# vb000/LookOnceToHear

Measured on AMD Instinct MI355X. Metric: frames_per_sec (5 s 16 kHz binaural clips, 625 STFT frames each, offline forward), higher is better.
Workload: dtype f32 via f16x3 split (3x fp16 MFMA per product, fp32 accumulate; ~22-bit operands, un-normalised rows scaled by a power of two before the split: any finite fp32 range); 1 GPU; BASELINE configs[2]: 32 x 5 s 16 kHz binaural clips per GPU, offline forward (configs/tsh.json separator, random-init weights); batch_per_gpu=32, global_batch=32, parallelism=utterance-dp1, gemm_mode=f16x3, tune=, batches_in_flight=1

## Files before the change

### include/lookonce_hip.h

```cpp
#ifndef LOOKONCE_HIP_H
#define LOOKONCE_HIP_H

#ifdef __cplusplus
extern "C" {
#endif

typedef void* lh_stream_t;

enum {
    LH_OK = 0,
    LH_ERR_ARG = 1,
    LH_ERR_UNSUPPORTED = 2,
    LH_ERR_LAUNCH = 3,
    LH_ERR_RANGE = 4
};

int lh_range_status(unsigned* range_flag, lh_stream_t stream);
int lh_range_flag_copy(unsigned* range_flag, void* host_pinned, lh_stream_t stream);
int lh_range_flag_clear(unsigned* range_flag, lh_stream_t stream);
int lh_selftest_fp16_subnormal(lh_stream_t stream);

enum { LH_GEMM_F32 = 0, LH_GEMM_F16X3 = 1 };

int lh_abi_version(void);

int lh_set_tuning(int key, int value);

int lh_check_config(int nfft, int hop, int n_mics, int emb_dim, int n_blocks_unused, int lstm_hidden,
                    int n_heads, int attn_window, int n_srcs, int spk_emb_dim);

int lh_stft_conv_in(const float* x, const float* conv_buf_in, float* conv_buf_out, const void* wfb_pk,
                    const void* wconv_pk, const float* bconv, float* z, int B, int T, int n_samples,
                    lh_stream_t stream);

int lh_embed_proj_ln(const float* emb, const float* w, const float* bias, const float* ln_w, const float* ln_b,
                     float* scratch, float* gain, int B, lh_stream_t stream);

int lh_ln_lstm_intra(const float* x, const float* ln_w, const float* ln_b, const void* w_pk, const float* b_sum,
                     float* h_out, int n_frames , int mode, lh_stream_t stream);

int lh_ln_lstm_inter(const float* x, const float* ln_w, const float* ln_b, const void* w_pk, const float* b_sum,
                     const float* h0, const float* c0, float* hN, float* cN, float* h_out, int B, int T, int mode,
                     lh_stream_t stream);

int lh_intra_stream(const float* x, const void* wih_pk, const float* b_sum, const float* whh, float* h_out,
                    int n_frames, lh_stream_t stream);

int lh_inter_matvec(const float* x, const void* wih_pk, const float* b_sum, const float* whh, const void* wlin_pk,
                    const float* blin, const float* h0, const float* c0, float* hN, float* cN, float* out, int B, int T,
                    lh_stream_t stream);

int lh_intra_block(const float* x, const void* w_pk, const float* b_sum, const void* wlin_pk, const float* blin,
                   float* out, int n_frames, lh_stream_t stream);

int lh_inter_block(const float* x, const void* w_pk, const float* b_sum, const void* wlin_pk, const float* blin,
                   const float* h0, const float* c0, float* hN, float* cN, float* out, int B, int T,
                   lh_stream_t stream);

int lh_linear_res(const float* h, const void* w_pk, const float* bias, const float* res, float* out, int rows,
                  int K, lh_stream_t stream);

#define LH_KV_PAD_ROWS 48

int lh_qkv_proj_ln(const float* y, const void* w_pk, const float* bias, const float* slopes, const float* lnq_w,
                   const float* lnq_b, const float* lnk_w, const float* lnk_b, const float* lnv_w,
                   const float* lnv_b, void* q, void* kx, void* vx, const int* ring_pos, int B, int T,
                   lh_stream_t stream);

int lh_qkv_proj_ln_rows(const float* y, const void* w_pk, const float* bias, const float* slopes, const float* lnq_w,
                        const float* lnq_b, const float* lnk_w, const float* lnk_b, const float* lnv_w,
                        const float* lnv_b, void* q, void* kx, void* vx, const int* write_pos, int B,
                        lh_stream_t stream);

int lh_local_attn(const void* q, const void* kx, const void* vx, float* merged, int B, int T, lh_stream_t stream);

int lh_ring_pack(const float* k_buf, const float* v_buf, void* kx, void* vx, int B, int T, lh_stream_t stream);
// ... 173 lines not shown
```

### lookoncetohear_amd/_cabi.py

```python
from __future__ import annotations

import ctypes
import os
from ctypes import c_double, c_int, c_ulonglong, c_void_p

_PKG = os.path.dirname(os.path.abspath(__file__))
HIP_LIB_PATH = os.path.join(_PKG, "_lookonce_hip.so")
ABI_VERSION = 23

_P, _I = c_void_p, c_int
SIGNATURES = {
    "lh_abi_version": [],
    "lh_check_config": [_I] * 10,
    "lh_stft_conv_in": [_P] * 7 + [_I] * 3 + [_P],
    "lh_embed_proj_ln": [_P] * 7 + [_I, _P],
    "lh_set_tuning": [_I, _I],
    "lh_ln_lstm_intra": [_P] * 6 + [_I, _I, _P],
    "lh_ln_lstm_inter": [_P] * 10 + [_I, _I, _I, _P],
    "lh_intra_stream": [_P] * 5 + [_I, _P],
    "lh_inter_matvec": [_P] * 11 + [_I, _I, _P],
    "lh_intra_block": [_P] * 6 + [_I, _P],
    "lh_inter_block": [_P] * 10 + [_I, _I, _P],
    "lh_linear_res": [_P] * 5 + [_I, _I, _P],
    "lh_qkv_proj_ln": [_P] * 14 + [_I, _I, _P],
    "lh_local_attn": [_P] * 4 + [_I, _I, _P],
    "lh_ring_pack": [_P] * 4 + [_I, _I, _P],
    "lh_ring_unpack": [_P] * 4 + [_I, _I, _P],
    "lh_ring_advance": [_P, _I, _P],
    "lh_session_begin": [_P, _I, _P, _P, _P, _P, _I, _P],
    "lh_session_end": [_P, _I, _P, _P, _P, _P, _P, _I, _P],
    "lh_session_capture": [_P] * 5 + [_I, _I, _P],
    "lh_session_move": [_P, _I, _P, _P, _P, _I, _I, _P],
    "lh_session_begin_rows": [_P, _I, _P, _P, _P, _P, _P, _I, _I, _P],
    "lh_session_end_rows": [_P, _I] + [_P] * 9 + [_I, _I, _P],
    "lh_qkv_proj_ln_rows": [_P] * 14 + [_I, _P],
    "lh_ring_advance_rows": [_P, _P, _I, _I, _P],
    "lh_session_begin_paced": [_P, _I] + [_P] * 7 + [_I, _P],
    "lh_session_end_paced": [_P, _I, _P, _I] + [_P] * 6 + [_I, _P],
    "lh_session_move_paced": [_P, _I, _P, _P, _P, _P, _I, _I, _P],
    "lh_session_begin_rows_paced": [_P, _I] + [_P] * 8 + [_I, _I, _P],
    "lh_session_end_rows_paced": [_P, _I, _P, _I] + [_P] * 10 + [_I, _I, _P],
    "lh_session_capture_paced": [_P] * 6 + [_I, _I, _P],
    "lh_session_save": [_P, _I, _P, _I, _I, _I, _I, _P, _I, _P, c_ulonglong, _P, _P, _P, _I, _I, _P],
    "lh_session_restore": [_P, _I, _P, _I, _I, _I, _I, _P, _I, _P, c_ulonglong, _P, _P, _P, _P, _I, _I, _I, _P],
# ... 151 lines not shown
```

### lookoncetohear_amd/csrc/lh_attn.hip

```cpp
#include "lh_common.h"

namespace lh {

typedef _Float16 f16x8 __attribute__((ext_vector_type(8)));
typedef _Float16 f16x4 __attribute__((ext_vector_type(4)));
struct Frag { f16x8 h, l; };
struct VQuad { f16x4 h, l; };

constexpr int AT_KSTEPS = (DQKP + 31) / 32;
constexpr int AT_PKS = 3;
constexpr int AT_PP = AT_PKS * 32 + 8;
constexpr int AT_CG = (DV + 63) / 64;

#if defined(LH_PROBE_TRACE)
__device__ unsigned long long lh_attn_trace_buf[16];
#define AT_STAMP(k) do { if (blockIdx.x == 803 && blockIdx.y == 0 && tid == 0) lh_attn_trace_buf[k] = __builtin_amdgcn_s_memtime(); } while (0)
#else
#define AT_STAMP(k) do { } while (0)
#endif
template <int MQ, int RING, int TQ = 16 * MQ>
__global__ void __launch_bounds__(256, 2) k_local_attn(const _Float16* __restrict__ q, const _Float16* __restrict__ kx,
                                                       const _Float16* __restrict__ vx, float* __restrict__ merged,
                                                       int BH, int T, int ntt, int tw0, int tend) {
    constexpr int NKEYS = TQ + HIST;
    constexpr int NKT = (NKEYS + 15) / 16;
    constexpr int NK = NKT * 16;
    constexpr int ND = 5;
    constexpr int NB = ND * 16;
    static_assert(TQ <= 16 * MQ && TQ > 16 * (MQ - 1) && NKEYS <= AT_PKS * 32 && NK - 1 <= HIST + KV_PAD, "tile geometry");
    __shared__ float sp[4][TQ][NB];
    __shared__ __attribute__((aligned(16))) _Float16 ph[16 * MQ][AT_PP];
    __shared__ __attribute__((aligned(16))) _Float16 pl[16 * MQ][AT_PP];
    const int tid = threadIdx.x, lane = tid & 63, wave = wave_id(tid), g4 = lane >> 4, l15 = lane & 15;
    const int xcd = blockIdx.x & 7, kk = blockIdx.x >> 3;
    const int bh = (kk / ntt) * 8 + xcd;
    const int t0 = tw0 + (kk % ntt) * TQ;
    if (bh >= BH) return;
    const long TKP = T + HIST + KV_PAD;
    const _Float16* qb = q + (long)bh * T * LDQKH;
    const _Float16* kb = kx + ((long)bh * TKP + t0) * LDQKH;
    const _Float16* vb = vx + ((long)bh * TKP + t0) * LDVH;

    AT_STAMP(0);
    {
        f32x4 am[MQ][ND];
#pragma unroll
        for (int mq = 0; mq < MQ; ++mq)
#pragma unroll
            for (int d = 0; d < ND; ++d) am[mq][d] = f32x4{0.f, 0.f, 0.f, 0.f};
        int qoff[MQ], koff[NKT];
#pragma unroll
        for (int mq = 0; mq < MQ; ++mq) qoff[mq] = min(t0 + mq * 16 + l15, tend - 1) * LDQKH + g4 * 16;
#pragma unroll
        for (int nt = 0; nt < NKT; ++nt) koff[nt] = (nt * 16 + l15) * LDQKH + g4 * 16;
        constexpr int NIT = (AT_KSTEPS + 3) / 4;
        Frag fq[2][MQ], fk[2][NKT];
        auto fetch = [&](int it, Frag (&dq)[MQ], Frag (&dk)[NKT]) {
            const int s = min(wave + 4 * it, AT_KSTEPS - 1);
#pragma unroll
// ... 243 lines not shown
    if (v < 0 || v > 3) return LH_ERR_ARG;
    g_attn_mq = v;
    return LH_OK;
}

}

extern "C" int lh_local_attn_win(const void* q, const void* kx, const void* vx, float* merged, int B, int T, int t0, int Tc,
                                 lh_stream_t stream) {
    using namespace lh;
    if (!q || !kx || !vx || !merged || B <= 0 || T <= 0 || t0 < 0 || Tc <= 0 || t0 + Tc > T) return LH_ERR_ARG;
    const int Tfull = T;
    const int Tshape = T;
    T = Tc;
    const int BH = B * NH;
    const int bh8 = (BH + 7) / 8 * 8;
    int mq = g_attn_mq;
    if (Tshape <= 16) mq = 1;
    else if (mq == 0) mq = (long)bh8 * ((Tshape + 31) / 32) > 512 ? 3 : 2;
    const int tq = mq == 3 ? 40 : 16 * mq;
    const int ntt = (T + tq - 1) / tq;
    const dim3 grid(bh8 * ntt, bh8 * ntt <= 64 ? 7 : 1);
    const _Float16 *qh = (const _Float16*)q, *kh = (const _Float16*)kx, *vh = (const _Float16*)vx;
    if (mq == 1)
        hipLaunchKernelGGL((k_local_attn<1, 3>), grid, dim3(256), 0, (hipStream_t)stream, qh, kh, vh, merged, BH, Tfull, ntt, t0, t0 + Tc);
    else if (mq == 3)
        hipLaunchKernelGGL((k_local_attn<3, 2, 40>), grid, dim3(256), 0, (hipStream_t)stream, qh, kh, vh, merged, BH, Tfull, ntt, t0, t0 + Tc);
    else
        hipLaunchKernelGGL((k_local_attn<2, 2>), grid, dim3(256), 0, (hipStream_t)stream, qh, kh, vh, merged, BH, Tfull, ntt, t0, t0 + Tc);
    return check_launch();
}

extern "C" int lh_local_attn(const void* q, const void* kx, const void* vx, float* merged, int B, int T,
                             lh_stream_t stream) {
    return lh_local_attn_win(q, kx, vx, merged, B, T, 0, T, stream);
}

extern "C" int lh_ring_pack(const float* k_buf, const float* v_buf, void* kx, void* vx, int B, int T,
                            lh_stream_t stream) {
    using namespace lh;
    if (!k_buf || !v_buf || !kx || !vx || B <= 0 || T <= 0) return LH_ERR_ARG;
    const int BH = B * NH;
    const long n = (long)BH * HIST * (QKB + DV / 4);
    const int grid = (int)((n + 255) / 256 < 2048 ? (n + 255) / 256 : 2048);
    hipLaunchKernelGGL(k_ring_pack, dim3(grid), dim3(256), 0, (hipStream_t)stream, k_buf, v_buf, (_Float16*)kx,
                       (_Float16*)vx, (long)T + HIST + KV_PAD, BH);
    return check_launch();
}

namespace lh {
__global__ void k_ring_advance(int* pos, int modulo) {
    const int p = *pos + 1;
// ... 40 lines not shown
```

### lookoncetohear_amd/csrc/lh_common.h

```cpp
#pragma once
#include <hip/hip_runtime.h>
#include <type_traits>
#include <utility>
#include "../../include/lookonce_hip.h"

namespace lh {

constexpr int NFFT = 192;
constexpr int HOP = 128;
constexpr int NF = 97;
constexpr int NK = 2 * NF;
constexpr int NMIC = 2;
constexpr int NSRC = 2;
constexpr int C = 64;
constexpr int H = 64;
constexpr int NH = 4;
constexpr int E = 6;
constexpr int VD = 16;
constexpr int DQK = NF * E;
constexpr int DV = NF * VD;
constexpr int QKB = 76;
constexpr int DQKP = QKB * 8;
constexpr int LDQKH = QKB * 16;
constexpr int LDVH = DV * 2;
// ... 147 lines not shown
    _Float16 h0, l0, h1, l1;
    split_hl(v0, h0, l0);
    split_hl(v1, h1, l1);
    hi = f16x2_t{h0, h1};
    lo = f16x2_t{l0, l1};
#endif
}

__device__ __forceinline__ void pin_here(float4& v) {
#if defined(__AMDGCN__)
    asm volatile("" : "+v"(v.x), "+v"(v.y), "+v"(v.z), "+v"(v.w));
#else
    (void)v;
#endif
}

template <class F, int... I>
__device__ __forceinline__ void xp_sf(F& f, std::integer_sequence<int, I...>) { (f(std::integral_constant<int, I>{}), ...); }
template <int N, class F>
__device__ __forceinline__ void xp_for(F&& f) { xp_sf(f, std::make_integer_sequence<int, N>{}); }

inline int check_launch() { return hipGetLastError() == hipSuccess ? LH_OK : LH_ERR_LAUNCH; }

}
```

### lookoncetohear_amd/csrc/lh_lstm.hip

```cpp
#include <type_traits>

#include "lh_common.h"

namespace lh {

constexpr int LS_PAD = 36;

template <int MT>
__global__ void __launch_bounds__(256) k_ln_lstm(const float* __restrict__ x, const float* __restrict__ lnw,
                                                 const float* __restrict__ lnb, const float* __restrict__ w_pk,
                                                 const float* __restrict__ b_sum, const float* __restrict__ h0,
                                                 const float* __restrict__ c0, float* __restrict__ hN,
                                                 float* __restrict__ cN, float* __restrict__ h_out, int nseq,
                                                 int nstep, int sdiv, int so, int si, int ps, int ldh) {
    constexpr int NS = 16 * MT;
    __shared__ __attribute__((aligned(16))) float abuf[2 * 4 * NS * LS_PAD];
    const int tid = threadIdx.x, lane = tid & 63, wave = wave_id(tid);
    const int dir = blockIdx.y;
    const int s0 = blockIdx.x * NS;
    const int g4 = lane >> 4, l15 = lane & 15;

    auto A = [&](int buf, int chunk, int row, int j) -> float* {
        return &abuf[((buf * 4 + chunk) * NS + row) * LS_PAD + j];
    };
// ... 885 lines not shown
    if (n == 0) {
        int dev = 0, v = 0;
        if (hipGetDevice(&dev) == hipSuccess &&
            hipDeviceGetAttribute(&v, hipDeviceAttributeMultiprocessorCount, dev) == hipSuccess && v > 0)
            n = v;
        else
            n = 256;
    }
    return n;
}
int emb_set(int key, int value);
static int g_tune[8] = {0, 0, 0, 0, 0, 0, 0, 0};
}
namespace lh { int attn_set_mq(int v); }
namespace lh {
int launch_intra_xp(const float* x, const void* w_pk, const float* b_sum, const void* wlin_pk, const float* blin, float* out,
                    int nseq, int nstep, int sdiv, int so, int si, int ps, int dir, int accumulate, hipStream_t st);
int xp_set(int key, int v);
int launch_inter_xp(const float* x, const void* w_pk, const float* b_sum, const void* wlin_pk, const float* blin,
                    const float* h0, const float* c0, float* hN, float* cN, float* out, int nseq, int nstep, int sdiv, int so,
                    int si, int ps, hipStream_t st, int cflags = 0);
}
namespace lh { int backend_set_runs(int v); }
namespace lh { int snap_set_tiles(int v); }
#if defined(LH_PROBE_TRACE)
extern "C" int lh_probe_trace_read(unsigned long long* host_dst) {
    return hipMemcpyFromSymbol(host_dst, HIP_SYMBOL(lh::lh_trace_buf), sizeof(lh::lh_trace_buf)) == hipSuccess ? 0 : 1;
}
#endif
extern "C" int lh_set_tuning(int key, int value) {
    if (key == 4) return lh::attn_set_mq(value);
    if (key == 6) return lh::backend_set_runs(value);
    if (key >= 7 && key < 16) return lh::xp_set(key, value);
    if (key == 16 || key == 17) return lh::emb_set(key, value);
    if (key == 18) return lh::snap_set_tiles(value);
    if (key < 0 || key >= 8) return LH_ERR_ARG;
#if defined(LH_LEGACY)
    if (key == 3) lh::g_dephase = value;
#else
    if (key == 2 && value == 2) return LH_ERR_UNSUPPORTED;
#endif
    lh::g_tune[key] = value;
    return LH_OK;
}

extern "C" int lh_ln_lstm_intra(const float* x, const float* ln_w, const float* ln_b, const void* w_pk,
                                const float* b_sum, float* h_out, int n_frames, int mode, lh_stream_t stream) {
    using namespace lh;
    if (!x || !ln_w || !ln_b || !w_pk || !b_sum || !h_out || n_frames <= 0) return LH_ERR_ARG;
    const int mt = g_tune[0] ? g_tune[0] : (mode == LH_GEMM_F16X3 ? 0 : (n_frames >= 8192 ? 2 : 1));
    if (mode == LH_GEMM_F16X3) {
        hipStream_t st = (hipStream_t)stream;
        if (mt == 2)
            return launch_lstm_h3<2>(x, ln_w, ln_b, w_pk, b_sum, nullptr, nullptr, nullptr, nullptr, h_out, n_frames, NF,
                                     2, 1, NF, 0, 1, 2 * H, st);
        if (mt == 1)
            return launch_lstm_h3<1>(x, ln_w, ln_b, w_pk, b_sum, nullptr, nullptr, nullptr, nullptr, h_out, n_frames, NF,
                                     2, 1, NF, 0, 1, 2 * H, st);
// ... 32 lines not shown
                                float* h_out, int B, int T, int mode, lh_stream_t stream) {
    using namespace lh;
    if (!x || !ln_w || !ln_b || !w_pk || !b_sum || !h0 || !c0 || !hN || !cN || !h_out || B <= 0 || T <= 0)
        return LH_ERR_ARG;
    if (h0 == hN || c0 == cN) return LH_ERR_ARG;
    const int nseq = B * NF;
    const int mt = g_tune[1] == 2 ? 2 : 1;
    if (mode == LH_GEMM_F16X3) {
        if (mt == 2)
            return launch_lstm_h3<2>(x, ln_w, ln_b, w_pk, b_sum, h0, c0, hN, cN, h_out, nseq, T, 1, NF, T * NF, 1, NF, H,
                                     (hipStream_t)stream);
        return launch_lstm_h3<1>(x, ln_w, ln_b, w_pk, b_sum, h0, c0, hN, cN, h_out, nseq, T, 1, NF, T * NF, 1, NF, H,
                                 (hipStream_t)stream);
    }
    if (mode != LH_GEMM_F32) return LH_ERR_UNSUPPORTED;
    const float* w_f32 = (const float*)w_pk;
    if (mt == 2)
        return launch_lstm<2>(x, ln_w, ln_b, w_f32, b_sum, h0, c0, hN, cN, h_out, nseq, T, 1, NF, T * NF, 1, NF, H,
                              (hipStream_t)stream);
    return launch_lstm<1>(x, ln_w, ln_b, w_f32, b_sum, h0, c0, hN, cN, h_out, nseq, T, 1, NF, T * NF, 1, NF, H,
                          (hipStream_t)stream);
}

extern "C" int lh_intra_block(const float* x, const void* w_pk, const float* b_sum, const void* wlin_pk,
                              const float* blin, float* out, int n_frames, lh_stream_t stream) {
    using namespace lh;
    if (!x || !w_pk || !b_sum || !wlin_pk || !blin || !out || n_frames <= 0 || x == out) return LH_ERR_ARG;
    hipStream_t st = (hipStream_t)stream;
    int rc = LH_OK;
    for (int dir = 0; dir < 2 && rc == LH_OK; ++dir)
#if defined(LH_LEGACY)
        if (g_tune[2] == 2)
            rc = launch_lstm_lin<1>(x, w_pk, b_sum, (const _Float16*)wlin_pk + (long)dir * 4 * 2 * 64 * 16, blin, nullptr, nullptr,
                                    nullptr, nullptr, out, n_frames, NF, 1, NF, 0, 1, dir, dir, st);
        else
#endif
            rc = launch_intra_xp(x, w_pk, b_sum, (const _Float16*)wlin_pk + (long)dir * 4 * 2 * 64 * 16, blin, out, n_frames,
                                 NF, 1, NF, 0, 1, dir, dir, st);
    return rc;
}

extern "C" int lh_intra_block_win(const float* x, const void* w_pk, const float* b_sum, const void* wlin_pk,
                                  const float* blin, float* out, int B, int T, int t0, int Tc, lh_stream_t stream) {
    using namespace lh;
    if (!x || !w_pk || !b_sum || !wlin_pk || !blin || !out || B <= 0 || T <= 0 || x == out || t0 < 0 || Tc <= 0 || t0 + Tc > T)
        return LH_ERR_ARG;
// ... 34 lines not shown
```

### lookoncetohear_amd/csrc/lh_pointwise.hip

```cpp
#include "lh_split.h"
#include <type_traits>

namespace lh {

template <int K>
__global__ void __launch_bounds__(256) k_linear_res(const float* __restrict__ h, const _Float16* __restrict__ w_pk,
                                                    const float* __restrict__ bias, const float* __restrict__ res,
                                                    float* __restrict__ out, int rows, int seg, long segstride) {
    auto grow = [&](long r) -> long { return (r / seg) * segstride + r % seg; };
    constexpr int KS = K / 32, RP = 64, CP = C + 4;
    __shared__ __attribute__((aligned(16))) _Float16 ahi[KS * 4 * RP * 8];
    __shared__ __attribute__((aligned(16))) _Float16 alo[KS * 4 * RP * 8];
    __shared__ __attribute__((aligned(16))) float cs[RP * CP];
    const int tid = threadIdx.x, lane = tid & 63, wave = wave_id(tid), g4 = lane >> 4, l15 = lane & 15;

    f16x8 wh[KS], wl[KS];
    load_w<KS>(w_pk, wave, lane, wh, wl);
    const float bz = bias[wave * 16 + l15];

    const int ntiles = (rows + RP - 1) / RP;
    for (int tile = blockIdx.x; tile < ntiles; tile += gridDim.x) {
        const long r0 = (long)tile * RP;
        constexpr int NLD = RP * (K / 4) / 256;
        float4 stg[NLD];
// ... 152 lines not shown
                const f32x4 c0 = s == 0 ? f32x4{0.f, 0.f, 0.f, 0.f} : r0[cur];
                r0[cur] = __builtin_amdgcn_mfma_f32_16x16x32_f16(av, j == 1 ? wl0[ks] : wh0[ks], c0, 0, 0, 0);
                if (TWO) {
                    const f32x4 c1 = s == 0 ? f32x4{0.f, 0.f, 0.f, 0.f} : r1[cur];
                    r1[cur] = __builtin_amdgcn_mfma_f32_16x16x32_f16(av, j == 1 ? wl1[ks] : wh1[ks], c1, 0, 0, 0);
                }
                if (m > 0 && s >= 1 && s <= 4) epilogue(std::integral_constant<int, s - 1>{});
                __builtin_amdgcn_sched_barrier(0);
            });
        } else if (g4 == 0) {
            epilogue(std::integral_constant<int, 0>{});
        }
    });
}

template <bool ROWS>
__global__ void __launch_bounds__(256, 2) k_qkv_proj_ln(const float* __restrict__ y, const _Float16* __restrict__ w_pk,
                                                     const float* __restrict__ bias, const float* __restrict__ slopes,
                                                     const float* __restrict__ lnq_w, const float* __restrict__ lnq_b,
                                                     const float* __restrict__ lnk_w, const float* __restrict__ lnk_b,
                                                     const float* __restrict__ lnv_w, const float* __restrict__ lnv_b,
                                                     _Float16* __restrict__ q, _Float16* __restrict__ kx,
                                                     _Float16* __restrict__ vx, int T, int nframes,
                                                     const int* __restrict__ ring_pos, int Tc, int tw0) {
    auto gidx = [&](int fr) -> long { return (long)(fr / Tc) * T + tw0 + fr % Tc; };
    __shared__ __attribute__((aligned(16))) _Float16 ahi[FR_A];
    __shared__ __attribute__((aligned(16))) _Float16 alo[FR_A];
    __shared__ __attribute__((aligned(16))) float yf[Y_N];
    __shared__ __attribute__((aligned(16))) float rinv[FR_RP];
    const int tid = threadIdx.x, lane = tid & 63, wave = wave_id(tid), g4 = lane >> 4, l15 = lane & 15;

    f16x8 wh0[2], wl0[2], wh1[2], wl1[2];
    load_w<2>(w_pk, wave, lane, wh0, wl0);
    const bool two = wave + 4 < NQKV / 16;
    load_w<2>(w_pk, two ? wave + 4 : wave, lane, wh1, wl1);
    const int c0 = wave * 16 + l15, c1 = c0 + 64;
    const float bz0 = bias[c0], bz1 = bias[two ? c1 : c0];
    const float sq = slopes[0], sk = slopes[1], sv = slopes[2];
    const float a0 = c0 < NH * E ? sq : (c0 < 2 * NH * E ? sk : sv);
    const bool le1 = sq <= 1.0f && sk <= 1.0f && sv <= 1.0f;
    int base0;
    if (c0 < NH * E) base0 = (c0 / E) * YQS + c0 % E;
    else if (c0 < 2 * NH * E) base0 = Y_K0 + ((c0 - NH * E) / E) * YQS + (c0 - NH * E) % E;
    else base0 = Y_V0 + ((c0 - 2 * NH * E) / VD) * DV + (c0 - 2 * NH * E) % VD;
    const int cv = (two ? c1 : c0) - 2 * NH * E;
    const int base1 = Y_V0 + (cv / VD) * DV + cv % VD;

    frame_zero_pad(ahi, alo, tid);
    if (tid < FR_RP - NF) rinv[NF + tid] = 0.f;
    for (int i = tid; i < 2 * NH * (YQS - DQK); i += 256)
        yf[(i / (YQS - DQK)) * YQS + DQK + i % (YQS - DQK)] = 0.f;
    HeadLN<DQK, 2 * QKB> aq, ak;
    aq.load_affine(lnq_w, lnq_b, lane);
    ak.load_affine(lnk_w, lnk_b, lane);
    float4 stg[FR_NLD];
    if ((int)blockIdx.x < nframes) frame_load(y + gidx(blockIdx.x) * NF * C, tid, stg);
    const long tkp = T + HIST + KV_PAD;
    const int krow0 = ROWS ? 0 : ring_pos ? (int)((unsigned)*ring_pos % (unsigned)WIN) : HIST;
    for (int fr = blockIdx.x; fr < nframes; fr += gridDim.x) {
        const int b = fr / Tc, t = tw0 + fr % Tc;
        QKV_STAMP(0);
        frame_store_scaled(ahi, alo, rinv, tid, stg);
        __syncthreads();
        QKV_STAMP(1);
        if (fr + (int)gridDim.x < nframes) frame_load(y + gidx(fr + gridDim.x) * NF * C, tid, stg);

        if (two) {
            if (le1) qkv_products<true, true>(ahi, alo, rinv, yf, g4, l15, wh0, wl0, wh1, wl1, bz0, bz1, a0, sv, base0, base1);
            else qkv_products<true, false>(ahi, alo, rinv, yf, g4, l15, wh0, wl0, wh1, wl1, bz0, bz1, a0, sv, base0, base1);
        } else {
            if (le1) qkv_products<false, true>(ahi, alo, rinv, yf, g4, l15, wh0, wl0, wh1, wl1, bz0, bz1, a0, sv, base0, base1);
            else qkv_products<false, false>(ahi, alo, rinv, yf, g4, l15, wh0, wl0, wh1, wl1, bz0, bz1, a0, sv, base0, base1);
        }
        QKV_STAMP(2);
        __syncthreads();
        QKV_STAMP(3);

        const int hd = wave;
        const long bh = (long)b * NH + hd;
        float* yq = yf + hd * YQS;
        float* yk = yf + Y_K0 + hd * YQS;
        float* yv = yf + Y_V0 + hd * DV;
        const float* zero8 = yf + DQKP - 8;
// ... 19 lines not shown
            HeadLN<DV, DV / 4> lv;
            lv.load_affine(lnv_w, lnv_b, ln);
            const float sv1 = lv.read(yv, zero8, ln);
            const float mv = wave_sum(sv1) * (1.0f / DV);
            const float vv = lv.center(mv, ln);
            const float rv = rsqrtf(wave_sum(vv) * (1.0f / DV) + LN_EPS);
            lv.store<1>(rv, vrow, ln);
        }
        QKV_STAMP(5);
    }
}
#if defined(LH_PROBE_TRACE)
}
extern "C" int lh_probe_qkv_trace_read(unsigned long long* host_dst) {
    return hipMemcpyFromSymbol(host_dst, HIP_SYMBOL(lh::lh_qkv_trace_buf), sizeof(lh::lh_qkv_trace_buf)) == hipSuccess ? 0 : 1;
}
namespace lh {
#endif

#if defined(LH_DBG_K6)
__device__ unsigned lh_dbg_k6[4];
__device__ float lh_dbg_part[8 * 24 * 256 * 4];
#endif
__global__ void __launch_bounds__(256, 2) k_proj_ln_res(const float* __restrict__ merged, const _Float16* __restrict__ w_pk,
                                                     const float* __restrict__ bias, const float* __restrict__ slope,
                                                     const float* __restrict__ lnw, const float* __restrict__ lnb,
                                                     const float* __restrict__ y2, const float* __restrict__ gain,
                                                     float* __restrict__ out, int T, int nframes, int Tc, int tw0) {
    constexpr int YP = C + 4;
    auto gidx = [&](int fr) -> long { return (long)(fr / Tc) * T + tw0 + fr % Tc; };
    __shared__ __attribute__((aligned(16))) _Float16 ahi[FR_A];
    __shared__ __attribute__((aligned(16))) _Float16 alo[FR_A];
    __shared__ __attribute__((aligned(16))) float ys[NF * YP];
    __shared__ float red[4];
    const int tid = threadIdx.x, lane = tid & 63, wave = wave_id(tid), g4 = lane >> 4, l15 = lane & 15;

    f16x8 wh[2], wl[2];
    load_w<2>(w_pk, wave, lane, wh, wl);
    const float bz = bias[wave * 16 + l15];
    const float a = slope[0];
    constexpr int N = NF * C, N4 = N / 4;
    constexpr int NSLOT = (N4 + 255) / 256;
    float4 pw[NSLOT], pb[NSLOT];
#pragma unroll
    for (int k = 0; k < NSLOT; ++k) {
        const int i = min(tid + 256 * k, N4 - 1);
        pw[k] = *reinterpret_cast<const float4*>(&lnw[i * 4]);
        pb[k] = *reinterpret_cast<const float4*>(&lnb[i * 4]);
    }

    frame_zero_pad(ahi, alo, tid);
    float4 stg[FR_NLD];
    if ((int)blockIdx.x < nframes) frame_load_heads(merged + gidx(blockIdx.x) * N, tid, stg);
    for (int fidx = blockIdx.x; fidx < nframes; fidx += gridDim.x) {
        const int b = fidx / Tc;
        const long fr = gidx(fidx) * N;
        frame_store(ahi, alo, tid, stg);
        __syncthreads();
        if (fidx + (int)gridDim.x < nframes) frame_load_heads(merged + gidx(fidx + gridDim.x) * N, tid, stg);

        float4 rv[NSLOT];
#pragma unroll
        for (int k = 0; k < NSLOT; ++k)
            rv[k] = *reinterpret_cast<const float4*>(&y2[fr + (long)min(tid + 256 * k, N4 - 1) * 4]);

        auto row_tile = [&](int m, auto checked, auto fast) {
            const f32x4 acc = mma_tile1<FR_RP, 2>(ahi, alo, m, g4, l15, wh, wl, bz);
#pragma unroll
            for (int r = 0; r < 4; ++r) {
                const int row = m * 16 + g4 * 4 + r;
                if (!checked.value || row < NF)
                    ys[row * YP + wave * 16 + l15] = fast.value ? prelu_mm<true>(acc[r], a) : prelu_f(acc[r], a);
            }
        };
        if (a <= 1.0f) {
#pragma unroll 1
            for (int m = 0; m < NF / 16; ++m) row_tile(m, std::false_type{}, std::true_type{});
            row_tile(NF / 16, std::true_type{}, std::true_type{});
        } else {
#pragma unroll 1
            for (int m = 0; m < NF / 16; ++m) row_tile(m, std::false_type{}, std::false_type{});
            row_tile(NF / 16, std::true_type{}, std::false_type{});
        }
        __syncthreads();

        float4 v[NSLOT];
        float s = 0.f;
// ... 76 lines not shown
    return launch_linear_res(h, w_pk, bias, res, out, rows, K, rows, 0L, (hipStream_t)stream);
}

extern "C" int lh_linear_res_win(const float* h, const void* w_pk, const float* bias, const float* res, float* out, int B, int T,
                                 int t0, int Tc, int K, lh_stream_t stream) {
    using namespace lh;
    if (!h || !w_pk || !bias || !res || !out || B <= 0 || T <= 0 || t0 < 0 || Tc <= 0 || t0 + Tc > T) return LH_ERR_ARG;
    const long off = (long)t0 * NF;
    return launch_linear_res(h + off * K, w_pk, bias, res + off * C, out + off * C, B * Tc * NF, K, Tc * NF, (long)T * NF,
                             (hipStream_t)stream);
}

extern "C" int lh_qkv_proj_ln_win(const float* y, const void* w_pk, const float* bias, const float* slopes,
                                  const float* lnq_w, const float* lnq_b, const float* lnk_w, const float* lnk_b,
                                  const float* lnv_w, const float* lnv_b, void* q, void* kx, void* vx, const int* ring_pos,
                                  int B, int T, int t0, int Tc, lh_stream_t stream) {
    using namespace lh;
    if (!y || !w_pk || !bias || !slopes || !lnq_w || !lnq_b || !lnk_w || !lnk_b || !lnv_w || !lnv_b || !q || !kx ||
        !vx || B <= 0 || T <= 0 || (ring_pos && T != 1) || t0 < 0 || Tc <= 0 || t0 + Tc > T)
        return LH_ERR_ARG;
    const int nframes = B * Tc;
    hipLaunchKernelGGL(k_qkv_proj_ln<false>, dim3(nframes < 512 ? nframes : 512), dim3(256), 0, (hipStream_t)stream, y,
                       (const _Float16*)w_pk, bias, slopes, lnq_w, lnq_b, lnk_w, lnk_b, lnv_w, lnv_b, (_Float16*)q,
                       (_Float16*)kx, (_Float16*)vx, T, nframes, ring_pos, Tc, t0);
    return check_launch();
}

extern "C" int lh_qkv_proj_ln(const float* y, const void* w_pk, const float* bias, const float* slopes,
                              const float* lnq_w, const float* lnq_b, const float* lnk_w, const float* lnk_b,
                              const float* lnv_w, const float* lnv_b, void* q, void* kx, void* vx, const int* ring_pos,
                              int B, int T, lh_stream_t stream) {
    return lh_qkv_proj_ln_win(y, w_pk, bias, slopes, lnq_w, lnq_b, lnk_w, lnk_b, lnv_w, lnv_b, q, kx, vx, ring_pos, B, T, 0, T,
                              stream);
}

extern "C" int lh_qkv_proj_ln_rows(const float* y, const void* w_pk, const float* bias, const float* slopes,
                                   const float* lnq_w, const float* lnq_b, const float* lnk_w, const float* lnk_b,
                                   const float* lnv_w, const float* lnv_b, void* q, void* kx, void* vx, const int* write_pos,
                                   int B, lh_stream_t stream) {
    using namespace lh;
    if (!y || !w_pk || !bias || !slopes || !lnq_w || !lnq_b || !lnk_w || !lnk_b || !lnv_w || !lnv_b || !q || !kx || !vx ||
        !write_pos || B <= 0)
        return LH_ERR_ARG;
    hipLaunchKernelGGL(k_qkv_proj_ln<true>, dim3(B < 512 ? B : 512), dim3(256), 0, (hipStream_t)stream, y,
                       (const _Float16*)w_pk, bias, slopes, lnq_w, lnq_b, lnk_w, lnk_b, lnv_w, lnv_b, (_Float16*)q,
                       (_Float16*)kx, (_Float16*)vx, 1, B, write_pos, 1, 0);
    return check_launch();
}

extern "C" int lh_proj_ln_res_win(const float* merged, const void* w_pk, const float* bias, const float* slope,
                                  const float* ln_w, const float* ln_b, const float* y2, const float* gain, float* out,
                                  int B, int T, int t0, int Tc, lh_stream_t stream) {
    using namespace lh;
    if (!merged || !w_pk || !bias || !slope || !ln_w || !ln_b || !y2 || !out || B <= 0 || T <= 0 || t0 < 0 || Tc <= 0 ||
        t0 + Tc > T)
        return LH_ERR_ARG;
    const int nframes = B * Tc;
    hipLaunchKernelGGL(k_proj_ln_res, dim3(nframes < 512 ? nframes : 512), dim3(256), 0, (hipStream_t)stream, merged,
                       (const _Float16*)w_pk, bias, slope, ln_w, ln_b, y2, gain, out, T, nframes, Tc, t0);
    return check_launch();
}

extern "C" int lh_proj_ln_res(const float* merged, const void* w_pk, const float* bias, const float* slope,
                              const float* ln_w, const float* ln_b, const float* y2, const float* gain, float* out,
                              int B, int T, lh_stream_t stream) {
    return lh_proj_ln_res_win(merged, w_pk, bias, slope, ln_w, ln_b, y2, gain, out, B, T, 0, T, stream);
}

#if defined(LH_DBG_K6)
extern "C" int lh_dbg_part_read(float* host) {
    return hipMemcpyFromSymbol(host, HIP_SYMBOL(lh::lh_dbg_part), sizeof(lh::lh_dbg_part)) == hipSuccess ? 0 : 1;
}
extern "C" int lh_dbg_k6_read(unsigned* host4, int reset) {
    if (hipMemcpyFromSymbol(host4, HIP_SYMBOL(lh::lh_dbg_k6), 16) != hipSuccess) return 1;
    if (reset) { unsigned z[4] = {0, 0, 0, 0}; (void)hipMemcpyToSymbol(HIP_SYMBOL(lh::lh_dbg_k6), z, 16); }
    return 0;
}
#endif
```

### lookoncetohear_amd/csrc/lh_recur.hip

```cpp
#include <tuple>
#include <type_traits>
#include <utility>

#include "lh_common.h"

namespace lh {

typedef _Float16 xp_f16x8 __attribute__((ext_vector_type(8)));
typedef _Float16 xp_f16x4 __attribute__((ext_vector_type(4)));
constexpr int XP_AP = 144;
constexpr int XP_LSP = 68;
constexpr float XP_K2 = -2.0f * LOG2E;

template <int NSLOT, class MF, class Ops>
__device__ __forceinline__ void xp_zip(MF& mf, Ops& ops) {
    constexpr int NOPS = (int)std::tuple_size<Ops>::value;
    xp_for<NSLOT>([&](auto s_) {
        constexpr int i = decltype(s_)::value;
        mf(s_);
        constexpr int a = i * NOPS / NSLOT, b = (i + 1) * NOPS / NSLOT;
        xp_for<b - a>([&](auto k_) { std::get<a + decltype(k_)::value>(ops)(); });
#if !defined(XP_NO_FENCE)
        __builtin_amdgcn_sched_barrier(0);
#endif
// ... 24 lines not shown
__device__ __forceinline__ float xp_exp2(float v) {
#if defined(XP_PROBE_NOTRANS)
    return __builtin_fmaf(v, 0.25f, 0.5f);
#else
    return __builtin_amdgcn_exp2f(v);
#endif
}
__device__ __forceinline__ float xp_rcp(float v) {
#if defined(XP_PROBE_NOTRANS)
    return __builtin_fmaf(v, -0.25f, 1.0f);
#else
    return __builtin_amdgcn_rcpf(v);
#endif
}
#if defined(XP_PROBE_HIHI)
constexpr int XP_NP = 1;
#else
constexpr int XP_NP = 3;
#endif

__global__ void __launch_bounds__(256, 2) k_intra_xp(const float* __restrict__ x, const _Float16* __restrict__ w_pk,
                                                     const float* __restrict__ b_sum, const _Float16* __restrict__ wlin_pk,
                                                     const float* __restrict__ blin, float* out, int nseq, int nstep,
                                                     int sdiv, int so, int si, int ps, int dir, int accumulate, int prio) {
    constexpr int NS = 16;
    __shared__ __attribute__((aligned(16))) _Float16 ahi[2 * NS * XP_AP];
    __shared__ __attribute__((aligned(16))) _Float16 alo[2 * NS * XP_AP];
    __shared__ __attribute__((aligned(16))) float ls[2 * NS * XP_LSP];
    const int tid = threadIdx.x, lane = tid & 63, wave = wave_id(tid);
#if defined(XP_TRACE)
    __shared__ unsigned long long tr[128 * 4];
    const int tr_slot = blockIdx.x == 7 ? 0 : (blockIdx.x == gridDim.x / 2 + 3 ? 1 : -1);
    const bool tr_on = tr_slot >= 0 && threadIdx.x == 0 && dir == 0;
    const unsigned long long wg_t0 = __builtin_amdgcn_s_memtime();
#endif
    if (prio == 1) {
        const unsigned hw_id = __builtin_amdgcn_s_getreg((4 - 1) << 11 | 0 << 6 | 4);
        if (hw_id & 1) __builtin_amdgcn_s_setprio(2);
    }
#if defined(LH_PROBE_INTRA1)
    const int nt1 = (nseq + NS - 1) / NS;
    dir = (int)blockIdx.x >= nt1;
    accumulate = dir;
    wlin_pk += (long)dir * 4 * 2 * 64 * 16;
    const int s0 = ((int)blockIdx.x - dir * nt1) * NS;
#else
    const int s0 = blockIdx.x * NS;
#endif
    const int g4 = lane >> 4, l15 = lane & 15;
    const int q = tid & 15;
    const int unit = wave * 16 + l15;

    auto row_of0 = [&](int s) -> long { return (long)(s / sdiv) * so + (long)(s % sdiv) * si; };
    const long wg_row0 = row_of0(min(s0, nseq - 1));
    const int srow = min(s0 + (tid >> 4), nseq - 1);
    const unsigned voff = (unsigned)((row_of0(srow) - wg_row0) * (C * 4) + q * 16);
    const char* xb = reinterpret_cast<const char*>(x) + wg_row0 * (C * 4);
    char* ob = reinterpret_cast<char*>(out) + wg_row0 * (C * 4);
    const char* bsrc = reinterpret_cast<const char*>(
        accumulate ? reinterpret_cast<unsigned long long>(ob) : reinterpret_cast<unsigned long long>(xb));
    const long step_bytes = (long)ps * (C * 4);
    auto step_pos = [&](int it) -> int { it = min(max(it, 0), nstep - 1); return dir ? (nstep - 1 - it) : it; };

    xp_f16x8 wh[4][4], wl[4][4];
    {
        const _Float16* wp = w_pk + ((long)(dir * 4 + wave) * 16 * 64 + lane) * 16;
#pragma unroll
        for (int g = 0; g < 4; ++g)
#pragma unroll
            for (int ks = 0; ks < 4; ++ks) {
// ... 608 lines not shown
static int g_xp_prio_inter = 3;

int launch_inter_xp(const float* x, const void* w_pk, const float* b_sum, const void* wlin_pk, const float* blin,
                    const float* h0, const float* c0, float* hN, float* cN, float* out, int nseq, int nstep, int sdiv, int so,
                    int si, int ps, hipStream_t st, int cflags) {
    if (nstep < 2) return LH_ERR_ARG;
    hipLaunchKernelGGL(k_inter_xp, dim3((nseq + 15) / 16), dim3(512), 0, st, x, (const _Float16*)w_pk, b_sum,
                       (const _Float16*)wlin_pk, blin, h0, c0, hN, cN, out, nseq, nstep, sdiv, so, si, ps, 0, 0, g_xp_prio_inter,
                       cflags);
    return check_launch();
}
int xp_set(int key, int v) {
    if (key == 7) g_xp_lds_pad = v < 0 ? 0 : v;
    if (key == 8) g_xp_prio = v;
    if (key == 9) g_xp_prio_inter = v;
    return LH_OK;
}

int launch_intra_xp(const float* x, const void* w_pk, const float* b_sum, const void* wlin_pk, const float* blin, float* out,
                    int nseq, int nstep, int sdiv, int so, int si, int ps, int dir, int accumulate, hipStream_t st) {
#if defined(LH_PROBE_INTRA1)
    if (dir == 1) return LH_OK;
    hipLaunchKernelGGL(k_intra_xp, dim3(2 * ((nseq + 15) / 16)), dim3(256), g_xp_lds_pad, st, x, (const _Float16*)w_pk, b_sum,
                       (const _Float16*)wlin_pk, blin, out, nseq, nstep, sdiv, so, si, ps, dir, accumulate, g_xp_prio);
    return check_launch();
#endif
    hipLaunchKernelGGL(k_intra_xp, dim3((nseq + 15) / 16), dim3(256), g_xp_lds_pad, st, x, (const _Float16*)w_pk, b_sum,
                       (const _Float16*)wlin_pk, blin, out, nseq, nstep, sdiv, so, si, ps, dir, accumulate, g_xp_prio);
    return check_launch();
}

}

#if defined(XP_TRACE)
extern "C" int lh_probe_xp_trace_inter_read(unsigned long long* host_dst) {
    return hipMemcpyFromSymbol(host_dst, HIP_SYMBOL(lh::xp_trace_inter), sizeof(lh::xp_trace_inter)) == hipSuccess ? 0 : 1;
}
extern "C" int lh_probe_xp_trace_read(unsigned long long* host_dst) {
    return hipMemcpyFromSymbol(host_dst, HIP_SYMBOL(lh::xp_trace_buf), sizeof(lh::xp_trace_buf)) == hipSuccess ? 0 : 1;
}
extern "C" int lh_probe_xp_wglog_read(unsigned long long* host_dst) {
    return hipMemcpyFromSymbol(host_dst, HIP_SYMBOL(lh::xp_wg_log), sizeof(lh::xp_wg_log)) == hipSuccess ? 0 : 1;
}
#endif
```

### lookoncetohear_amd/csrc/lh_split.h

```cpp
#pragma once
#include "lh_common.h"

namespace lh {

typedef _Float16 f16x8 __attribute__((ext_vector_type(8)));
typedef _Float16 f16x4 __attribute__((ext_vector_type(4)));

template <int RP>
__device__ __forceinline__ int a_slot(int blk, int row) { return (blk * RP + (row ^ (blk & 7))) * 8; }
template <int RP>
__device__ __forceinline__ int a_index(int row, int k) {
    return a_slot<RP>((k >> 5) * 4 + ((k >> 3) & 3), row) + (k & 7);
}

template <int RP>
__device__ __forceinline__ void store_split4(_Float16* ahi, _Float16* alo, int row, int k0, float4 v) {
    f16x2_t h01, l01, h23, l23;
    split_pair(v.x, v.y, h01, l01);
    split_pair(v.z, v.w, h23, l23);
    const f16x4 h4 = f16x4{h01[0], h01[1], h23[0], h23[1]}, l4 = f16x4{l01[0], l01[1], l23[0], l23[1]};
    const int idx = a_index<RP>(row, k0);
    *reinterpret_cast<f16x4*>(&ahi[idx]) = h4;
    *reinterpret_cast<f16x4*>(&alo[idx]) = l4;
}
// ... 43 lines not shown

template <int KS>
__device__ __forceinline__ void load_w(const _Float16* __restrict__ w_pk, int nt, int lane, f16x8 (&wh)[KS],
                                       f16x8 (&wl)[KS]) {
#pragma unroll
    for (int ks = 0; ks < KS; ++ks) {
        const _Float16* p = w_pk + ((long)(nt * KS + ks) * 64 + lane) * 16;
        wh[ks] = *reinterpret_cast<const f16x8*>(p);
        wl[ks] = *reinterpret_cast<const f16x8*>(p + 8);
    }
}

constexpr int FR_RP = 112;
constexpr int FR_A = 2 * 4 * FR_RP * 8;
constexpr int FR_NLD = (NF * 16 + 255) / 256;

__device__ __forceinline__ void frame_load(const float* __restrict__ src, int tid, float4 (&stg)[FR_NLD]) {
#pragma unroll
    for (int i = 0; i < FR_NLD; ++i) {
        const int e = min(tid + 256 * i, NF * 16 - 1);
        stg[i] = *reinterpret_cast<const float4*>(&src[(e >> 4) * C + (e & 15) * 4]);
    }
}
__device__ __forceinline__ void frame_load_heads(const float* __restrict__ src, int tid, float4 (&stg)[FR_NLD]) {
#pragma unroll
    for (int i = 0; i < FR_NLD; ++i) {
        const int e = min(tid + 256 * i, NF * 16 - 1);
        stg[i] = *reinterpret_cast<const float4*>(&src[((e & 15) >> 2) * DV + (e >> 4) * VD + (e & 3) * 4]);
    }
}
__device__ __forceinline__ void frame_store(_Float16* ahi, _Float16* alo, int tid, const float4 (&stg)[FR_NLD]) {
#pragma unroll
    for (int i = 0; i < FR_NLD; ++i) {
        const int e = tid + 256 * i;
        if (e < NF * 16) store_split4<FR_RP>(ahi, alo, e >> 4, (e & 15) * 4, stg[i]);
    }
}
constexpr int FR_TE = 12;
__device__ __forceinline__ void frame_store_scaled(_Float16* ahi, _Float16* alo, float* rinv, int tid,
                                                   const float4 (&stg)[FR_NLD]) {
    float m = 0.f;
#pragma unroll
    for (int i = 0; i < FR_NLD; ++i) m = fmaxf(m, absmax4(stg[i]));
    float s, inv;
    pow2_scale<FR_TE>(wave_max_uniform(m), s, inv);
#pragma unroll
    for (int i = 0; i < FR_NLD; ++i) {
        const int e = tid + 256 * i;
        if (e < NF * 16) {
            store_split4<FR_RP>(ahi, alo, e >> 4, (e & 15) * 4, make_float4(stg[i].x * s, stg[i].y * s, stg[i].z * s, stg[i].w * s));
            if ((e & 15) == 0) rinv[e >> 4] = inv;
// ... 10 lines not shown
```

Measured before the change: 2.911 million frames/s.

## Reorder block visit order across kernels for cache locality and add nontemporal loads

Adds a tunable visit-order bitmask, on by default with value 17 (intra tiles plus nontemporal flag). The intra LSTM kernel now visits tiles in a residue-grouped order and walks backward for the reverse direction. QKV, attention and projection kernels gain optional batch-interleaved frame orders, which are off by default. The projection kernel uses nontemporal loads when its working set exceeds 256 MB. The aim is better L2/MALL reuse between producer and consumer kernels and less cache pollution from streaming reads, at the cost of extra index arithmetic per block.

```diff
diff --git a/include/lookonce_hip.h b/include/lookonce_hip.h
--- a/include/lookonce_hip.h
+++ b/include/lookonce_hip.h
@@ -24,6 +24,7 @@
 
 int lh_abi_version(void);
 
+#define LH_VISIT_ORDER_DEFAULT 17
 int lh_set_tuning(int key, int value);
 
 int lh_check_config(int nfft, int hop, int n_mics, int emb_dim, int n_blocks_unused, int lstm_hidden,
@@ -52,6 +53,8 @@
 
 int lh_intra_block(const float* x, const void* w_pk, const float* b_sum, const void* wlin_pk, const float* blin,
                    float* out, int n_frames, lh_stream_t stream);
+
+int lh_intra_tile_order(int nseq, int Tc, int* tiles_out);
 
 int lh_inter_block(const float* x, const void* w_pk, const float* b_sum, const void* wlin_pk, const float* blin,
                    const float* h0, const float* c0, float* hN, float* cN, float* out, int B, int T,
diff --git a/lookoncetohear_amd/_cabi.py b/lookoncetohear_amd/_cabi.py
--- a/lookoncetohear_amd/_cabi.py
+++ b/lookoncetohear_amd/_cabi.py
@@ -20,6 +20,7 @@
     "lh_intra_stream": [_P] * 5 + [_I, _P],
     "lh_inter_matvec": [_P] * 11 + [_I, _I, _P],
     "lh_intra_block": [_P] * 6 + [_I, _P],
+    "lh_intra_tile_order": [_I, _I, _P],
     "lh_inter_block": [_P] * 10 + [_I, _I, _P],
     "lh_linear_res": [_P] * 5 + [_I, _I, _P],
     "lh_qkv_proj_ln": [_P] * 14 + [_I, _I, _P],
diff --git a/lookoncetohear_amd/csrc/lh_attn.hip b/lookoncetohear_amd/csrc/lh_attn.hip
--- a/lookoncetohear_amd/csrc/lh_attn.hip
+++ b/lookoncetohear_amd/csrc/lh_attn.hip
@@ -21,7 +21,7 @@
 template <int MQ, int RING, int TQ = 16 * MQ>
 __global__ void __launch_bounds__(256, 2) k_local_attn(const _Float16* __restrict__ q, const _Float16* __restrict__ kx,
                                                        const _Float16* __restrict__ vx, float* __restrict__ merged,
-                                                       int BH, int T, int ntt, int tw0, int tend) {
+                                                       int BH, int T, int ntt, int tw0, int tend, int ord8) {
     constexpr int NKEYS = TQ + HIST;
     constexpr int NKT = (NKEYS + 15) / 16;
     constexpr int NK = NKT * 16;
@@ -33,8 +33,8 @@
     __shared__ __attribute__((aligned(16))) _Float16 pl[16 * MQ][AT_PP];
     const int tid = threadIdx.x, lane = tid & 63, wave = wave_id(tid), g4 = lane >> 4, l15 = lane & 15;
     const int xcd = blockIdx.x & 7, kk = blockIdx.x >> 3;
-    const int bh = (kk / ntt) * 8 + xcd;
-    const int t0 = tw0 + (kk % ntt) * TQ;
+    const int bh = (ord8 ? kk % ord8 : kk / ntt) * 8 + xcd;
+    const int t0 = tw0 + (ord8 ? kk / ord8 : kk % ntt) * TQ;
     if (bh >= BH) return;
     const long TKP = T + HIST + KV_PAD;
     const _Float16* qb = q + (long)bh * T * LDQKH;
@@ -324,12 +324,13 @@
     const int ntt = (T + tq - 1) / tq;
     const dim3 grid(bh8 * ntt, bh8 * ntt <= 64 ? 7 : 1);
     const _Float16 *qh = (const _Float16*)q, *kh = (const _Float16*)kx, *vh = (const _Float16*)vx;
+    const int ord8 = (visit_order() & ORD_ATTN) ? bh8 / 8 : 0;
     if (mq == 1)
-        hipLaunchKernelGGL((k_local_attn<1, 3>), grid, dim3(256), 0, (hipStream_t)stream, qh, kh, vh, merged, BH, Tfull, ntt, t0, t0 + Tc);
+        hipLaunchKernelGGL((k_local_attn<1, 3>), grid, dim3(256), 0, (hipStream_t)stream, qh, kh, vh, merged, BH, Tfull, ntt, t0, t0 + Tc, ord8);
     else if (mq == 3)
-        hipLaunchKernelGGL((k_local_attn<3, 2, 40>), grid, dim3(256), 0, (hipStream_t)stream, qh, kh, vh, merged, BH, Tfull, ntt, t0, t0 + Tc);
+        hipLaunchKernelGGL((k_local_attn<3, 2, 40>), grid, dim3(256), 0, (hipStream_t)stream, qh, kh, vh, merged, BH, Tfull, ntt, t0, t0 + Tc, ord8);
     else
-        hipLaunchKernelGGL((k_local_attn<2, 2>), grid, dim3(256), 0, (hipStream_t)stream, qh, kh, vh, merged, BH, Tfull, ntt, t0, t0 + Tc);
+        hipLaunchKernelGGL((k_local_attn<2, 2>), grid, dim3(256), 0, (hipStream_t)stream, qh, kh, vh, merged, BH, Tfull, ntt, t0, t0 + Tc, ord8);
     return check_launch();
 }
 
diff --git a/lookoncetohear_amd/csrc/lh_common.h b/lookoncetohear_amd/csrc/lh_common.h
--- a/lookoncetohear_amd/csrc/lh_common.h
+++ b/lookoncetohear_amd/csrc/lh_common.h
@@ -193,4 +193,36 @@
 
 inline int check_launch() { return hipGetLastError() == hipSuccess ? LH_OK : LH_ERR_LAUNCH; }
 
-}
+constexpr int ORD_INTRA = 1, ORD_QKV = 2, ORD_ATTN = 4, ORD_PROJ = 8, ORD_NT = 16, ORD_ALL = 31;
+int visit_order();
+template <bool NT>
+__device__ __forceinline__ float4 ld4(const void* p) {
+    if (NT) {
+        const f32x4 v = __builtin_nontemporal_load(reinterpret_cast<const f32x4*>(p));
+        return make_float4(v[0], v[1], v[2], v[3]);
+    }
+    return *reinterpret_cast<const float4*>(p);
+}
+
+__device__ __forceinline__ void frame_of(int fr, int Tc, int ordB, int& b, int& j) {
+    if (ordB) { b = fr % ordB; j = Tc - 1 - fr / ordB; }
+    else { b = fr / Tc; j = fr % Tc; }
+}
+
+__host__ __device__ inline int intra_tile_at(int rank, int nseq, int T) {
+    const int B = nseq / T, nlo = T / 16;
+    const int k = min(rank / B, nlo);
+    int idx = rank - k * B;
+    const int m = (16 - T % 16) % 16, d = m ? (m & -m) : 16, P = 16 / d;
+    for (int u = 0; u < P; ++u) {
+        const int r = d * u;
+        int c0 = 0;
+        while (((c0 * m) & 15) != r) ++c0;
+        const int n = c0 < B ? (B - c0 + P - 1) / P : 0;
+        if (idx < n) return (int)((((long)(c0 + idx * P)) * T + r + 16 * k) / 16);
+        idx -= n;
+    }
+    return rank;
+}
+
+}
diff --git a/lookoncetohear_amd/csrc/lh_lstm.hip b/lookoncetohear_amd/csrc/lh_lstm.hip
--- a/lookoncetohear_amd/csrc/lh_lstm.hip
+++ b/lookoncetohear_amd/csrc/lh_lstm.hip
@@ -931,6 +931,10 @@
                     int si, int ps, hipStream_t st, int cflags = 0);
 }
 namespace lh { int backend_set_runs(int v); }
+namespace lh {
+static int g_visit_order = LH_VISIT_ORDER_DEFAULT;
+int visit_order() { return g_visit_order; }
+}
 namespace lh { int snap_set_tiles(int v); }
 #if defined(LH_PROBE_TRACE)
 extern "C" int lh_probe_trace_read(unsigned long long* host_dst) {
@@ -943,6 +947,11 @@
     if (key >= 7 && key < 16) return lh::xp_set(key, value);
     if (key == 16 || key == 17) return lh::emb_set(key, value);
     if (key == 18) return lh::snap_set_tiles(value);
+    if (key == 19) {
+        if (value < 0 || value > lh::ORD_ALL) return LH_ERR_ARG;
+        lh::g_visit_order = value;
+        return LH_OK;
+    }
     if (key < 0 || key >= 8) return LH_ERR_ARG;
 #if defined(LH_LEGACY)
     if (key == 3) lh::g_dephase = value;
@@ -1021,6 +1030,12 @@
                           (hipStream_t)stream);
 }
 
+extern "C" int lh_intra_tile_order(int nseq, int Tc, int* tiles_out) {
+    if (!tiles_out || nseq <= 0 || Tc <= 0 || nseq % Tc) return LH_ERR_ARG;
+    for (int rank = 0; rank < (nseq + 15) / 16; ++rank) tiles_out[rank] = lh::intra_tile_at(rank, nseq, Tc);
+    return LH_OK;
+}
+
 extern "C" int lh_intra_block(const float* x, const void* w_pk, const float* b_sum, const void* wlin_pk,
                               const float* blin, float* out, int n_frames, lh_stream_t stream) {
     using namespace lh;
diff --git a/lookoncetohear_amd/csrc/lh_pointwise.hip b/lookoncetohear_amd/csrc/lh_pointwise.hip
--- a/lookoncetohear_amd/csrc/lh_pointwise.hip
+++ b/lookoncetohear_amd/csrc/lh_pointwise.hip
@@ -198,8 +198,8 @@
                                                      const float* __restrict__ lnv_w, const float* __restrict__ lnv_b,
                                                      _Float16* __restrict__ q, _Float16* __restrict__ kx,
                                                      _Float16* __restrict__ vx, int T, int nframes,
-                                                     const int* __restrict__ ring_pos, int Tc, int tw0) {
-    auto gidx = [&](int fr) -> long { return (long)(fr / Tc) * T + tw0 + fr % Tc; };
+                                                     const int* __restrict__ ring_pos, int Tc, int tw0, int ordB) {
+    auto gidx = [&](int fr) -> long { int b, j; frame_of(fr, Tc, ordB, b, j); return (long)b * T + tw0 + j; };
     __shared__ __attribute__((aligned(16))) _Float16 ahi[FR_A];
     __shared__ __attribute__((aligned(16))) _Float16 alo[FR_A];
     __shared__ __attribute__((aligned(16))) float yf[Y_N];
@@ -234,7 +234,9 @@
     const long tkp = T + HIST + KV_PAD;
     const int krow0 = ROWS ? 0 : ring_pos ? (int)((unsigned)*ring_pos % (unsigned)WIN) : HIST;
     for (int fr = blockIdx.x; fr < nframes; fr += gridDim.x) {
-        const int b = fr / Tc, t = tw0 + fr % Tc;
+        int b, t;
+        frame_of(fr, Tc, ordB, b, t);
+        t += tw0;
         QKV_STAMP(0);
         frame_store_scaled(ahi, alo, rinv, tid, stg);
         __syncthreads();
@@ -300,13 +302,14 @@
 __device__ unsigned lh_dbg_k6[4];
 __device__ float lh_dbg_part[8 * 24 * 256 * 4];
 #endif
+template <bool NT>
 __global__ void __launch_bounds__(256, 2) k_proj_ln_res(const float* __restrict__ merged, const _Float16* __restrict__ w_pk,
                                                      const float* __restrict__ bias, const float* __restrict__ slope,
                                                      const float* __restrict__ lnw, const float* __restrict__ lnb,
                                                      const float* __restrict__ y2, const float* __restrict__ gain,
-                                                     float* __restrict__ out, int T, int nframes, int Tc, int tw0) {
+                                                     float* __restrict__ out, int T, int nframes, int Tc, int tw0, int ordB) {
     constexpr int YP = C + 4;
-    auto gidx = [&](int fr) -> long { return (long)(fr / Tc) * T + tw0 + fr % Tc; };
+    auto gidx = [&](int fr) -> long { int b, j; frame_of(fr, Tc, ordB, b, j); return (long)b * T + tw0 + j; };
     __shared__ __attribute__((aligned(16))) _Float16 ahi[FR_A];
     __shared__ __attribute__((aligned(16))) _Float16 alo[FR_A];
     __shared__ __attribute__((aligned(16))) float ys[NF * YP];
@@ -329,18 +332,19 @@
 
     frame_zero_pad(ahi, alo, tid);
     float4 stg[FR_NLD];
-    if ((int)blockIdx.x < nframes) frame_load_heads(merged + gidx(blockIdx.x) * N, tid, stg);
+    if ((int)blockIdx.x < nframes) frame_load_heads<NT>(merged + gidx(blockIdx.x) * N, tid, stg);
     for (int fidx = blockIdx.x; fidx < nframes; fidx += gridDim.x) {
-        const int b = fidx / Tc;
-        const long fr = gidx(fidx) * N;
+        int b, j;
+        frame_of(fidx, Tc, ordB, b, j);
+        const long fr = ((long)b * T + tw0 + j) * N;
         frame_store(ahi, alo, tid, stg);
         __syncthreads();
-        if (fidx + (int)gridDim.x < nframes) frame_load_heads(merged + gidx(fidx + gridDim.x) * N, tid, stg);
+        if (fidx + (int)gridDim.x < nframes) frame_load_heads<NT>(merged + gidx(fidx + gridDim.x) * N, tid, stg);
 
         float4 rv[NSLOT];
 #pragma unroll
         for (int k = 0; k < NSLOT; ++k)
-            rv[k] = *reinterpret_cast<const float4*>(&y2[fr + (long)min(tid + 256 * k, N4 - 1) * 4]);
+            rv[k] = ld4<NT>(&y2[fr + (long)min(tid + 256 * k, N4 - 1) * 4]);
 
         auto row_tile = [&](int m, auto checked, auto fast) {
             const f32x4 acc = mma_tile1<FR_RP, 2>(ahi, alo, m, g4, l15, wh, wl, bz);
@@ -463,7 +467,8 @@
     const int nframes = B * Tc;
     hipLaunchKernelGGL(k_qkv_proj_ln<false>, dim3(nframes < 512 ? nframes : 512), dim3(256), 0, (hipStream_t)stream, y,
                        (const _Float16*)w_pk, bias, slopes, lnq_w, lnq_b, lnk_w, lnk_b, lnv_w, lnv_b, (_Float16*)q,
-                       (_Float16*)kx, (_Float16*)vx, T, nframes, ring_pos, Tc, t0);
+                       (_Float16*)kx, (_Float16*)vx, T, nframes, ring_pos, Tc, t0,
+                       (visit_order() & ORD_QKV) && T > 1 ? B : 0);
     return check_launch();
 }
 
@@ -485,7 +490,7 @@
         return LH_ERR_ARG;
     hipLaunchKernelGGL(k_qkv_proj_ln<true>, dim3(B < 512 ? B : 512), dim3(256), 0, (hipStream_t)stream, y,
                        (const _Float16*)w_pk, bias, slopes, lnq_w, lnq_b, lnk_w, lnk_b, lnv_w, lnv_b, (_Float16*)q,
-                       (_Float16*)kx, (_Float16*)vx, 1, B, write_pos, 1, 0);
+                       (_Float16*)kx, (_Float16*)vx, 1, B, write_pos, 1, 0, 0);
     return check_launch();
 }
 
@@ -497,8 +502,14 @@
         t0 + Tc > T)
         return LH_ERR_ARG;
     const int nframes = B * Tc;
-    hipLaunchKernelGGL(k_proj_ln_res, dim3(nframes < 512 ? nframes : 512), dim3(256), 0, (hipStream_t)stream, merged,
-                       (const _Float16*)w_pk, bias, slope, ln_w, ln_b, y2, gain, out, T, nframes, Tc, t0);
+    const int ordB = (visit_order() & ORD_PROJ) ? B : 0;
+    const bool nt = (visit_order() & ORD_NT) && (long)nframes * NF * C * 4 > (256L << 20);
+    if (nt)
+        hipLaunchKernelGGL(k_proj_ln_res<true>, dim3(nframes < 512 ? nframes : 512), dim3(256), 0, (hipStream_t)stream, merged,
+                           (const _Float16*)w_pk, bias, slope, ln_w, ln_b, y2, gain, out, T, nframes, Tc, t0, ordB);
+    else
+        hipLaunchKernelGGL(k_proj_ln_res<false>, dim3(nframes < 512 ? nframes : 512), dim3(256), 0, (hipStream_t)stream, merged,
+                           (const _Float16*)w_pk, bias, slope, ln_w, ln_b, y2, gain, out, T, nframes, Tc, t0, ordB);
     return check_launch();
 }
 
diff --git a/lookoncetohear_amd/csrc/lh_recur.hip b/lookoncetohear_amd/csrc/lh_recur.hip
--- a/lookoncetohear_amd/csrc/lh_recur.hip
+++ b/lookoncetohear_amd/csrc/lh_recur.hip
@@ -70,7 +70,8 @@
 __global__ void __launch_bounds__(256, 2) k_intra_xp(const float* __restrict__ x, const _Float16* __restrict__ w_pk,
                                                      const float* __restrict__ b_sum, const _Float16* __restrict__ wlin_pk,
                                                      const float* __restrict__ blin, float* out, int nseq, int nstep,
-                                                     int sdiv, int so, int si, int ps, int dir, int accumulate, int prio) {
+                                                     int sdiv, int so, int si, int ps, int dir, int accumulate, int prio,
+                                                     int ord) {
     constexpr int NS = 16;
     __shared__ __attribute__((aligned(16))) _Float16 ahi[2 * NS * XP_AP];
     __shared__ __attribute__((aligned(16))) _Float16 alo[2 * NS * XP_AP];
@@ -93,7 +94,8 @@
     wlin_pk += (long)dir * 4 * 2 * 64 * 16;
     const int s0 = ((int)blockIdx.x - dir * nt1) * NS;
 #else
-    const int s0 = blockIdx.x * NS;
+    const int rank = dir ? (int)(gridDim.x - 1 - blockIdx.x) : (int)blockIdx.x;
+    const int s0 = (ord ? intra_tile_at(rank, nseq, sdiv) : (int)blockIdx.x) * NS;
 #endif
     const int g4 = lane >> 4, l15 = lane & 15;
     const int q = tid & 15;
@@ -748,11 +750,12 @@
 #if defined(LH_PROBE_INTRA1)
     if (dir == 1) return LH_OK;
     hipLaunchKernelGGL(k_intra_xp, dim3(2 * ((nseq + 15) / 16)), dim3(256), g_xp_lds_pad, st, x, (const _Float16*)w_pk, b_sum,
-                       (const _Float16*)wlin_pk, blin, out, nseq, nstep, sdiv, so, si, ps, dir, accumulate, g_xp_prio);
+                       (const _Float16*)wlin_pk, blin, out, nseq, nstep, sdiv, so, si, ps, dir, accumulate, g_xp_prio, 0);
     return check_launch();
 #endif
     hipLaunchKernelGGL(k_intra_xp, dim3((nseq + 15) / 16), dim3(256), g_xp_lds_pad, st, x, (const _Float16*)w_pk, b_sum,
-                       (const _Float16*)wlin_pk, blin, out, nseq, nstep, sdiv, so, si, ps, dir, accumulate, g_xp_prio);
+                       (const _Float16*)wlin_pk, blin, out, nseq, nstep, sdiv, so, si, ps, dir, accumulate, g_xp_prio,
+                       visit_order() & ORD_INTRA);
     return check_launch();
 }
 
diff --git a/lookoncetohear_amd/csrc/lh_split.h b/lookoncetohear_amd/csrc/lh_split.h
--- a/lookoncetohear_amd/csrc/lh_split.h
+++ b/lookoncetohear_amd/csrc/lh_split.h
@@ -89,11 +89,12 @@
         stg[i] = *reinterpret_cast<const float4*>(&src[(e >> 4) * C + (e & 15) * 4]);
     }
 }
+template <bool NT = false>
 __device__ __forceinline__ void frame_load_heads(const float* __restrict__ src, int tid, float4 (&stg)[FR_NLD]) {
 #pragma unroll
     for (int i = 0; i < FR_NLD; ++i) {
         const int e = min(tid + 256 * i, NF * 16 - 1);
-        stg[i] = *reinterpret_cast<const float4*>(&src[((e & 15) >> 2) * DV + (e >> 4) * VD + (e & 3) * 4]);
+        stg[i] = ld4<NT>(&src[((e & 15) >> 2) * DV + (e >> 4) * VD + (e & 3) * 4]);
     }
 }
 __device__ __forceinline__ void frame_store(_Float16* ahi, _Float16* alo, int tid, const float4 (&stg)[FR_NLD]) {
```

After: 2.930 million frames/s, median of 6. Within noise of the previous version (+0.7%).
